# ZhengmaoHe/PARC

Hardware: AMD Instinct MI355X
Metric: env-steps/sec (whole node), 4096 envs/GPU humanoid tracker at 1/2/4/8 MI355X (higher is better)
Workload: dtype f32; 1 GPU; 4096 envs/GPU tracker on procgen box heightfields, 64 synthetic clips (BASELINE.json configs[2]); envs_per_gpu=4096, env_steps_per_bench_step=131072, rollout_steps=32, update_epochs=5, minibatch=16384, sim_substeps=4, parallelism=dp1, scaling_rule=per-rank work fixed (T = 32, minibatch = 4 x envs): weak scaling, grad_allreduce=per minibatch (reference cadence)

## Files before the change

include/parc_hip.h:

```cpp
#ifndef PARC_HIP_H
#define PARC_HIP_H

#include <stdint.h>

#ifdef __cplusplus
extern "C" {
#endif

#define PARC_MAX_BODIES 16
#define PARC_MAX_DOFS 64
#define PARC_MAX_TAR_STEPS 6
#define PARC_MAX_KEY_BODIES 8

#define PARC_OK 0
#define PARC_EINVAL (-1)
#define PARC_EUNSUPPORTED (-2)

#define PARC_JOINT_ROOT 0
#define PARC_JOINT_HINGE 1
#define PARC_JOINT_SPHERICAL 2
#define PARC_JOINT_FIXED 3

#define PARC_DONE_NULL 0
#define PARC_DONE_FAIL 1
// ... 140 lines not shown
                               parc_track_cfg_t cfg, parc_env_buffers_t buf, const int64_t *env_ids, int n_sel, int what,
                               const float *ray_xy, void *start_event, void *stop_event);

int parc_assemble_obs(void *stream, int n_envs, const float *obs, int obs_dim, const float *aux, const float *scalar,
                      const int32_t *col_map, float *out, int out_dim, const int64_t *env_ids, int n_sel);

int parc_reset_apply(void *stream, int n_envs, const int32_t *mask, const int64_t *new_motion_ids, const int64_t *new_terrain_ids,
                     const float *new_time_offsets, const float *motion_offsets, int terrains_per_motion, int64_t *motion_ids,
                     int64_t *motion_terrain_ids, float *motion_time_offsets, float *motion_xy_offset, int32_t *timestep_buf,
                     float *time_buf, int32_t *done, float *next_target_time, int64_t *ep_num);

int parc_reset_sample_apply(void *stream, int n_envs, const int32_t *done_flags, int32_t *mask, const float *uniforms, int n_motions,
                            const float *motion_weights, const float *fail_rates, float min_weight, const float *motion_lengths,
                            const float *motion_offsets, int terrains_per_motion, float noise_scale, float *cdf_workspace,
                            int64_t *motion_ids, int64_t *motion_terrain_ids, float *motion_time_offsets, float *motion_xy_offset,
                            int32_t *timestep_buf, float *time_buf, int32_t *done, float *next_target_time, int64_t *ep_num,
                            float *init_noise_xy);

int parc_step_tail(void *stream, parc_char_model_t model, parc_motion_lib_t mlib, parc_env_buffers_t buf, int what, int n_motions,
                   const int32_t *done_kind, float ema_w, float *fail_rates);
int parc_update_fail_rates(void *stream, int n_envs, int n_motions, const int64_t *motion_ids, const int32_t *done_kind,
                           float ema_w, float *fail_rates);

int parc_td_lambda_return(void *stream, int T, int N, const float *reward, const float *next_vals, const int32_t *done,
                          float discount, float td_lambda, float *ret);
int parc_adv_normalize(void *stream, int n, const float *ret, const float *vals, const float *rand_action_mask,
                       float clip, float *norm_adv, float *mean_std_out , double *workspace);

typedef struct {
    float clip_ratio, bound_w, entropy_w, reg_w, critic_w, large_critic_loss;
    int32_t critic_l1;
} parc_ppo_cfg_t;
int parc_ppo_loss(void *stream, int B, int A, const float *mean, const float *logstd, const float *norm_a, const float *old_logp,
                  const float *adv, const float *mask, const float *pred, const float *tar_val, parc_ppo_cfg_t cfg, float *g_mean,
                  float *g_logstd, float *g_pred, float *out, float *workspace);
int parc_ppo_workspace_floats(int B);
int parc_ppo_loss_packed(void *stream, int B, int A, const float *mean, const float *logstd, const float *rec, int rec_stride,
                         const float *pred, parc_ppo_cfg_t cfg, float *g_mean, float *g_logstd, float *g_pred, float *out,
                         float *workspace);

typedef struct {
    const void *src;
    void *dst;
    int32_t row_bytes;
    int32_t convert;
} parc_record_field_t;
int parc_record_step(void *stream, int n_envs, const int64_t *head, int n_fields, const parc_record_field_t *fields);

int parc_rng_step(void *stream, uint64_t seed, uint64_t *state, float *uniform_out, int64_t n_uniform, float *normal_out, int64_t n_normal,
                  int64_t *tick_cell, int tick_mod);

int64_t parc_sgd_workspace_floats(void);
int parc_sgd_momentum_step(void *stream, int64_t n, float *params, const float *grad, float *momentum_buf, float max_norm, float lr,
                           float momentum, float weight_decay, float *workspace, float *norm_out);

int parc_adamw_step(void *stream, int64_t n, float *params, const float *grad, float *exp_avg, float *exp_avg_sq, int64_t step,
                    float max_norm, float lr, float beta1, float beta2, float eps, float weight_decay, float *workspace, float *norm_out);

int parc_normalize_clamp(void *stream, int64_t rows, int dim, const float *x, const float *mean, const float *stdv, float clip, float *out);

int64_t parc_moments_workspace_floats(int64_t rows, int dim);
int parc_moments_accumulate(void *stream, int64_t rows, int dim, const float *x, float *acc, float *workspace);
int parc_obs_ingest(void *stream, int64_t rows, int dim, const float *x, const float *mean, const float *stdv, float clip, float *norm_out,
                    float *copy_dst, const int64_t *copy_row, float *acc, float *workspace);

int parc_action_head(void *stream, int n, int A, const float *mean, const float *logstd, const float *noise, const float *explore,
                     const float *a_mean, const float *a_std, float *action, float *logp);
int parc_action_head_record(void *stream, int n, int A, const float *mean, const float *logstd, const float *noise, const float *explore,
                            const float *a_mean, const float *a_std, float *action, float *logp, float *rec_action, float *rec_logp,
                            float *rec_mask, const float *forces_src, float *rec_forces, int n_forces, const int64_t *head);

int parc_points_hf_sdf(void *stream, int batch, int n_points, int dim_x, int dim_y, const float *points, const float *hf,
                       const float *min_box_center, const float *x_points, const float *y_points, float half_x, float half_y,
                       float base_z, int inverted, float radius, float *out, int32_t *out_cell);

int parc_points_hf_sdf_grad(void *stream, int batch, int n_points, int dim_x, int dim_y, const float *points, const float *hf,
                            const float *min_box_center, const float *x_points, const float *y_points, float half_x, float half_y,
                            float base_z, int inverted, const int32_t *cell, const float *g_out, float *g_points);

int64_t parc_relu_bwd_workspace_floats(int64_t rows, int dim);
int parc_relu_bwd_bias_grad(void *stream, int64_t rows, int dim, float *gy, const float *y, float *db, float *workspace);
int parc_weighted_colsum(void *stream, int64_t rows, int dim, const float *x, const float *w, float *out, float *workspace);

int parc_abi_version(void);

#ifdef __cplusplus
}
#endif
#endif
```

parc_amd/_hip.py:

```python
import ctypes
import os
import subprocess

import torch

_HERE = os.path.dirname(os.path.abspath(__file__))
LIB_DIR = os.path.join(_HERE, "lib")
LIB_PATH = os.path.join(LIB_DIR, "libparc_hip.so")
CSRC = os.path.join(_HERE, "csrc")
SOURCES = ["parc_kin.hip", "parc_sim.hip", "parc_ppo.hip", "parc_rollout.hip", "parc_optim.hip", "parc_colreduce.hip", "parc_terrain.hip", "parc_render.hip", "parc_score.hip", "parc_netstats.hip", "parc_moopt.hip",
           "parc_augment.hip", "parc_mdm_batch.hip", "parc_hfgather.hip", "parc_motion.hip", "parc_pose_opt.hip", "parc_returns.hip"]
DIAG_LIB_PATH = os.path.join(LIB_DIR, "libparc_hip_diag.so")
DIAG_SOURCES = SOURCES + ["parc_sim_ref.hip"]

MAX_BODIES = 16
MAX_DOFS = 64
MAX_TAR_STEPS = 6
MAX_KEY_BODIES = 8

POST_REF = 1
POST_OBS = 2
POST_REWARD_DONE = 4
POST_HF = 8
POST_MASKED = 16
# ... 120 lines not shown
        objs.append(o)
    for cmd, p in procs:
        if p.wait() != 0:
            raise subprocess.CalledProcessError(p.returncode, cmd)
    cmd = [hipcc, "--offload-arch=gfx950", "-shared", "-fPIC", "-o", lib_path] + objs
    if verbose:
        print(" ".join(cmd))
    subprocess.check_call(cmd)
    with open(digest_path, "w") as f:
        f.write(digest + "\n")
    return lib_path


def lib():
    global _lib
    if _lib is None:
        if not os.path.exists(LIB_PATH):
            raise RuntimeError("libparc_hip.so is not built ({}); run `python -c 'import __graft_entry__ as g; g.build()'` "
                               "-- there is no CPU fallback".format(LIB_PATH))
        if _stored_digest() != source_digest():
            raise RuntimeError("libparc_hip.so was built from other sources than the ones beside it (csrc/, include/): rebuild with "
                               "`python -c 'import __graft_entry__ as g; g.build()'` - calling a stale library would hand it argument "
                               "structs of another layout")
        _lib = ctypes.CDLL(LIB_PATH)
        _declare(_lib)
    return _lib


def _declare(L):
    L.parc_abi_version.restype = c_int
    L.parc_refresh_ray_obs_hfs.argtypes = [c_vp, c_int, c_vp, c_int, c_vp, c_vp, TerrainS, c_f, c_f, c_vp, c_i64]
    L.parc_refresh_obs_hfs.argtypes = [c_vp, c_int, c_vp, c_int, c_vp, c_vp, TerrainS, c_f, c_f, c_vp, c_i64]
    L.parc_dof_to_rot.argtypes = [c_vp, CharModelS, c_int, c_vp, c_vp]
    L.parc_rot_to_dof.argtypes = [c_vp, CharModelS, c_int, c_vp, c_vp]
    L.parc_forward_kinematics.argtypes = [c_vp, CharModelS, c_int, c_vp, c_vp, c_vp, c_vp, c_vp]
    L.parc_pose_chain_forward.argtypes = [c_vp, CharModelS, c_int, c_vp, c_vp, c_vp, c_vp, c_vp, c_vp, c_vp]
    L.parc_pose_chain_backward.argtypes = [c_vp, CharModelS, c_int, c_vp, c_vp, c_vp, c_vp, c_vp, c_vp, c_vp, c_vp, c_vp]
    L.parc_body_points_world.argtypes = [c_vp, c_int, c_int, c_int, c_vp, c_vp, c_vp, c_vp, c_vp]
    L.parc_body_points_world_grad.argtypes = [c_vp, c_int, c_int, c_int, c_vp, c_vp, c_vp, c_vp, c_vp, c_vp]
    L.parc_quat_diff_angle.argtypes = [c_vp, ctypes.c_int64, c_vp, c_vp, c_vp]
    L.parc_quat_diff_angle_grad.argtypes = [c_vp, ctypes.c_int64, c_vp, c_vp, c_vp, c_vp, c_vp]
    L.parc_temporal_terms.argtypes = [c_vp, c_int, c_int, c_vp, c_vp, c_vp, c_vp, c_vp, c_f, c_f, c_f, c_vp]
    L.parc_temporal_terms_grad.argtypes = [c_vp, c_int, c_int, c_vp, c_vp, c_vp, c_vp, c_vp, c_f, c_f, c_f, c_vp, c_vp, c_vp]
    L.parc_calc_motion_frame.argtypes = [c_vp, MotionLibS, c_int, c_vp, c_vp] + [c_vp] * 7
    L.parc_motion_lib_build.argtypes = [c_vp, CharModelS, MotionLibS, c_int, c_vp, c_vp, c_vp, c_vp, c_vp]
    L.parc_track_post_step.argtypes = [c_vp, CharModelS, MotionLibS, TerrainS, TrackCfgS, EnvBuffersS, c_vp, c_int, c_int, c_vp]
    L.parc_track_post_step_timed.argtypes = L.parc_track_post_step.argtypes + [c_vp, c_vp]
    L.parc_track_post_step_timed.restype = c_int
    L.parc_assemble_obs.argtypes = [c_vp, c_int, c_vp, c_int, c_vp, c_vp, c_vp, c_vp, c_int, c_vp, c_int]
    L.parc_assemble_obs.restype = c_int
    L.parc_update_fail_rates.argtypes = [c_vp, c_int, c_int, c_vp, c_vp, c_f, c_vp]
    L.parc_step_tail.argtypes = [c_vp, CharModelS, MotionLibS, EnvBuffersS, c_int, c_int, c_vp, c_f, c_vp]
    L.parc_step_tail.restype = c_int
    L.parc_td_lambda_return.argtypes = [c_vp, c_int, c_int, c_vp, c_vp, c_vp, c_f, c_f, c_vp]
    L.parc_adv_normalize.argtypes = [c_vp, c_int, c_vp, c_vp, c_vp, c_f, c_vp, c_vp, c_vp]
    L.parc_ppo_loss.argtypes = [c_vp, c_int, c_int] + [c_vp] * 8 + [PPOCfgS] + [c_vp] * 5
    L.parc_ppo_loss.restype = c_int
    L.parc_ppo_loss_packed.argtypes = [c_vp, c_int, c_int, c_vp, c_vp, c_vp, c_int, c_vp, PPOCfgS] + [c_vp] * 5
    L.parc_ppo_loss_packed.restype = c_int
    L.parc_ppo_workspace_floats.argtypes = [c_int]
    L.parc_ppo_workspace_floats.restype = c_int
    L.parc_normalize_clamp.argtypes = [c_vp, c_i64, c_int, c_vp, c_vp, c_vp, c_f, c_vp]
    L.parc_normalize_clamp.restype = c_int
    L.parc_action_head.argtypes = [c_vp, c_int, c_int] + [c_vp] * 8
    L.parc_action_head.restype = c_int
    L.parc_action_head_record.argtypes = [c_vp, c_int, c_int] + [c_vp] * 8 + [c_vp] * 5 + [c_int, c_vp]
    L.parc_action_head_record.restype = c_int
    L.parc_points_hf_sdf.argtypes = [c_vp, c_int, c_int, c_int, c_int] + [c_vp] * 5 + [c_f, c_f, c_f, c_int, c_f, c_vp, c_vp]
    L.parc_points_hf_sdf.restype = c_int
    L.parc_points_hf_sdf_grad.argtypes = [c_vp, c_int, c_int, c_int, c_int] + [c_vp] * 5 + [c_f, c_f, c_f, c_int, c_vp, c_vp, c_vp]
    L.parc_points_hf_sdf_grad.restype = c_int
    L.parc_scale_by_clipped_norm.argtypes = [c_vp, c_i64, c_vp, c_vp, c_f]
    L.parc_scale_by_clipped_norm.restype = c_int
    L.parc_moments_workspace_floats.argtypes = [c_i64, c_int]
    L.parc_moments_workspace_floats.restype = c_i64
    L.parc_moments_accumulate.argtypes = [c_vp, c_i64, c_int, c_vp, c_vp, c_vp]
    L.parc_moments_accumulate.restype = c_int
    L.parc_relu_bwd_workspace_floats.argtypes = [c_i64, c_int]
    L.parc_relu_bwd_workspace_floats.restype = c_i64
    L.parc_relu_bwd_bias_grad.argtypes = [c_vp, c_i64, c_int, c_vp, c_vp, c_vp, c_vp]
    L.parc_relu_bwd_bias_grad.restype = c_int
    L.parc_weighted_colsum.argtypes = [c_vp, c_i64, c_int, c_vp, c_vp, c_vp, c_vp]
    L.parc_weighted_colsum.restype = c_int
    L.parc_sgd_workspace_floats.argtypes = []
    L.parc_sgd_workspace_floats.restype = c_i64
    L.parc_sgd_momentum_step.argtypes = [c_vp, c_i64, c_vp, c_vp, c_vp, c_f, c_f, c_f, c_f, c_vp, c_vp]
    L.parc_sgd_momentum_step.restype = c_int
    L.parc_adamw_step.argtypes = [c_vp, c_i64, c_vp, c_vp, c_vp, c_vp, c_i64, c_f, c_f, c_f, c_f, c_f, c_f, c_vp, c_vp]
    L.parc_adamw_step.restype = c_int
    L.parc_return_tracker_update.argtypes = [c_vp, c_int, c_int, c_vp, c_i64] + [c_vp] * 8
    L.parc_return_tracker_workspace_floats.argtypes = [c_int]
    L.parc_return_tracker_workspace_floats.restype = c_i64
    L.parc_return_tracker_update.restype = c_int
    L.parc_record_step.argtypes = [c_vp, c_int, c_vp, c_int, c_vp]
    L.parc_record_step.restype = c_int
    L.parc_obs_ingest.argtypes = [c_vp, c_i64, c_int, c_vp, c_vp, c_vp, c_f, c_vp, c_vp, c_vp, c_vp, c_vp]
    L.parc_obs_ingest.restype = c_int
    L.parc_rng_step.argtypes = [c_vp, ctypes.c_uint64, c_vp, c_vp, c_i64, c_vp, c_i64, c_vp, c_int]
    L.parc_rng_step.restype = c_int
    L.parc_reset_apply.argtypes = [c_vp, c_int, c_vp, c_vp, c_vp, c_vp, c_vp, c_int] + [c_vp] * 9
    L.parc_reset_apply.restype = c_int
    L.parc_reset_sample_apply.argtypes = [c_vp, c_int, c_vp, c_vp, c_vp, c_int, c_vp, c_vp, c_f, c_vp, c_vp, c_int, c_f] + [c_vp] * 11
    L.parc_reset_sample_apply.restype = c_int
    for name in ("parc_refresh_ray_obs_hfs", "parc_refresh_obs_hfs", "parc_dof_to_rot", "parc_rot_to_dof",
                 "parc_forward_kinematics", "parc_calc_motion_frame", "parc_motion_lib_build", "parc_track_post_step", "parc_reset_apply",
                 "parc_update_fail_rates", "parc_td_lambda_return", "parc_adv_normalize"):
        getattr(L, name).restype = c_int
    if hasattr(L, "parc_sim_abi"):
        from . import _hip_sim
        _hip_sim.declare(L)
    if hasattr(L, "parc_render_abi"):
        from . import _hip_render
        _hip_render.declare(L)
    if hasattr(L, "parc_score_abi"):
        from . import _hip_score
        _hip_score.declare(L)
    if hasattr(L, "parc_netstats_abi"):
        from . import _hip_netstats
        _hip_netstats.declare(L)
    if hasattr(L, "parc_moopt_abi"):
        from . import _hip_moopt
        _hip_moopt.declare(L)
    if hasattr(L, "parc_augment_abi"):
        from . import _hip_augment
        _hip_augment.declare(L)
    if hasattr(L, "parc_mdm_batch_abi"):
        from . import _hip_mdm_batch
        _hip_mdm_batch.declare(L)


EXPORTED = ["parc_abi_version", "parc_refresh_ray_obs_hfs", "parc_refresh_obs_hfs", "parc_dof_to_rot", "parc_rot_to_dof",
            "parc_forward_kinematics", "parc_calc_motion_frame", "parc_motion_lib_build", "parc_track_post_step",
            "parc_update_fail_rates", "parc_td_lambda_return", "parc_adv_normalize", "parc_reset_apply", "parc_ppo_loss", "parc_ppo_workspace_floats", "parc_record_step", "parc_return_tracker_update", "parc_normalize_clamp",
            "parc_action_head", "parc_points_hf_sdf", "parc_moments_workspace_floats", "parc_moments_accumulate", "parc_reset_sample_apply", "parc_return_tracker_workspace_floats", "parc_scale_by_clipped_norm", "parc_relu_bwd_workspace_floats",
            "parc_relu_bwd_bias_grad", "parc_ppo_loss_packed", "parc_weighted_colsum", "parc_sgd_workspace_floats", "parc_sgd_momentum_step", "parc_adamw_step",
            "parc_pose_chain_forward", "parc_pose_chain_backward", "parc_points_hf_sdf_grad", "parc_body_points_world", "parc_body_points_world_grad",
            "parc_quat_diff_angle", "parc_quat_diff_angle_grad", "parc_temporal_terms", "parc_temporal_terms_grad", "parc_step_tail",
            "parc_assemble_obs", "parc_track_post_step_timed", "parc_rng_step", "parc_obs_ingest", "parc_action_head_record",
            "parc_render", "parc_render_abi", "parc_motion_score", "parc_score_abi",
            "parc_netstats_workspace_floats", "parc_netstats_update", "parc_netstats_abs_colsum", "parc_netstats_dormant_count", "parc_netstats_abi",
            "parc_points_hf_sdf_ragged", "parc_points_hf_sdf_ragged_grad", "parc_temporal_terms_seg", "parc_temporal_terms_seg_grad",
            "parc_segment_sums", "parc_moopt_abi",
            "parc_augment_frames", "parc_augment_terrains", "parc_augment_localize", "parc_augment_abi",
            "parc_mdm_heightfields", "parc_mdm_windows", "parc_mdm_batch_abi"]


def check(rc, what):
    if rc != 0:
        raise RuntimeError("{} failed with code {} ({})".format(what, rc, "bad argument" if rc == -1 else "unsupported" if rc == -2 else "hipError"))


def stream():
    return c_vp(torch.cuda.current_stream().cuda_stream)


def ptr(t):
    if t is None:
        return c_vp(0)
    assert t.is_cuda, "HIP kernels need device tensors (no CPU fallback)"
    assert t.is_contiguous(), "tensor must be contiguous"
    return c_vp(t.data_ptr())


def terrain_struct(hf, min_point, dxdy):
    assert hf.dtype == torch.float32 and hf.is_contiguous() and hf.dim() == 2
    return TerrainS(ptr(hf), int(hf.shape[0]), int(hf.shape[1]), float(min_point[0]), float(min_point[1]),
                    float(dxdy[0]), float(dxdy[1]))


class HipEventPair:
    _rt = None

    def __init__(self):
        if HipEventPair._rt is None:
            HipEventPair._rt = ctypes.CDLL("libamdhip64.so")
        self.start, self.stop = c_vp(), c_vp()
        for ev in (self.start, self.stop):
            rc = HipEventPair._rt.hipEventCreate(ctypes.byref(ev))
            if rc != 0:
                raise RuntimeError("hipEventCreate -> %d" % rc)

    def elapsed_us(self):
        ms = ctypes.c_float()
        rc = HipEventPair._rt.hipEventElapsedTime(ctypes.byref(ms), self.start, self.stop)
        if rc != 0:
            raise RuntimeError("hipEventElapsedTime -> %d" % rc)
        return ms.value * 1e3

    def __del__(self):
        try:
            for ev in (self.start, self.stop):
                if ev:
                    HipEventPair._rt.hipEventDestroy(ev)
        except Exception:
            pass
```

parc_amd/csrc/parc_colreduce.hip:

```cpp
#include <hip/hip_runtime.h>
#include <stdint.h>

#include "../../include/parc_hip.h"
#include "parc_launch.h"
#include "parc_learner_math.h"

__global__ __launch_bounds__(256) void normalize_clamp_kernel(size_t n4, int dim4, const float4 *__restrict__ x, const float4 *__restrict__ mean,
                                                              const float4 *__restrict__ stdv, float clip, float4 *__restrict__ out) {
    for (size_t i = (size_t)blockIdx.x * blockDim.x + threadIdx.x; i < n4; i += (size_t)gridDim.x * blockDim.x) {
        const int c = (int)(i % (size_t)dim4);
        const float4 v = x[i], m = mean[c], s = stdv[c];
        float4 o;
        o.x = clamp_nan((v.x - m.x) / s.x, -clip, clip);
        o.y = clamp_nan((v.y - m.y) / s.y, -clip, clip);
        o.z = clamp_nan((v.z - m.z) / s.z, -clip, clip);
        o.w = clamp_nan((v.w - m.w) / s.w, -clip, clip);
        out[i] = o;
    }
}

extern "C" int parc_normalize_clamp(void *stream, int64_t rows, int dim, const float *x, const float *mean, const float *stdv, float clip,
                                    float *out) {
    if (rows < 0 || dim <= 0 || (dim & 3) || (((uintptr_t)x | (uintptr_t)mean | (uintptr_t)stdv | (uintptr_t)out) & 15)) return PARC_EINVAL;
    if (rows == 0) return PARC_OK;
// ... 138 lines not shown
    hipLaunchKernelGGL(moments_partial_kernel, g.grid, dim3(256), 0, (hipStream_t)stream, (int)rows, g.dim4, (const float4 *)x, (float4 *)workspace);
    launch_moments_final(stream, g, workspace, acc);
    PARC_CHECK_LAUNCH();
    return PARC_OK;
}

#define RB_ROWS 128
__global__ __launch_bounds__(256) void relu_bwd_bias_partial_kernel(int rows, int dim4, float4 *__restrict__ gy, const float4 *__restrict__ y,
                                                                    float4 *__restrict__ partial) {
    __shared__ float4 red[4][64];
    const col_chunk_t k = col_chunk(rows, RB_ROWS);
    const int rg = k.rg, c = k.c, r0 = k.r0, r1 = k.r1;
    float4 s = make_float4(0.f, 0.f, 0.f, 0.f);
    if (c < dim4) {
#pragma unroll 4
        for (int r = r0 + rg; r < r1; r += 4) {
            const size_t i = (size_t)r * dim4 + c;
            float4 g = gy[i];
            const float4 a = y[i];
            g.x = a.x <= 0.f ? 0.f : g.x; g.y = a.y <= 0.f ? 0.f : g.y; g.z = a.z <= 0.f ? 0.f : g.z; g.w = a.w <= 0.f ? 0.f : g.w;
            gy[i] = g;
            s.x += g.x; s.y += g.y; s.z += g.z; s.w += g.w;
        }
    }
    fold_store(red, s, k, dim4, partial);
}

__global__ __launch_bounds__(256) void colsum_final_kernel(int chunks, int dim, const float *__restrict__ partial, float *__restrict__ out) {
    const int c = blockIdx.x * blockDim.x + threadIdx.x;
    if (c >= dim) return;
    float t = 0.f;
#pragma unroll 16
    for (int k = 0; k < chunks; ++k) t += partial[(size_t)k * dim + c];
    out[c] = t;
}

__global__ __launch_bounds__(256) void weighted_colsum_partial_kernel(int rows, int dim4, const float4 *__restrict__ x, const float *__restrict__ w,
                                                                      float4 *__restrict__ partial) {
    __shared__ float4 red[4][64];
    const col_chunk_t k = col_chunk(rows, RB_ROWS);
    const int rg = k.rg, c = k.c, r0 = k.r0, r1 = k.r1;
    float4 s = make_float4(0.f, 0.f, 0.f, 0.f);
    if (c < dim4) {
#pragma unroll 4
        for (int r = r0 + rg; r < r1; r += 4) {
            const float4 v = x[(size_t)r * dim4 + c];
            const float wr = w[r];
            s.x = fmaf(wr, v.x, s.x); s.y = fmaf(wr, v.y, s.y); s.z = fmaf(wr, v.z, s.z); s.w = fmaf(wr, v.w, s.w);
        }
    }
    fold_store(red, s, k, dim4, partial);
}

static void launch_colsum_final(void *stream, const col_grid_t &g, int dim, const float *workspace, float *out) {
    hipLaunchKernelGGL(colsum_final_kernel, dim3((dim + 255) / 256), dim3(256), 0, (hipStream_t)stream, g.chunks, dim, workspace, out);
}

extern "C" int parc_weighted_colsum(void *stream, int64_t rows, int dim, const float *x, const float *w, float *out, float *workspace) {
    const col_grid_t g = col_chunk_grid(rows, dim, RB_ROWS, (uintptr_t)x | (uintptr_t)workspace, !x || !w || !out || !workspace);
    if (g.rc != PARC_OK) return g.rc;
    if (rows > 0)
        hipLaunchKernelGGL(weighted_colsum_partial_kernel, g.grid, dim3(256), 0, (hipStream_t)stream, (int)rows, g.dim4, (const float4 *)x, w,
                           (float4 *)workspace);
    launch_colsum_final(stream, g, dim, workspace, out);
    PARC_CHECK_LAUNCH();
    return PARC_OK;
}

extern "C" int64_t parc_relu_bwd_workspace_floats(int64_t rows, int dim) {
    if (rows < 0 || dim <= 0) return -1;
    return ((rows + RB_ROWS - 1) / RB_ROWS) * (int64_t)dim;
}

extern "C" int parc_relu_bwd_bias_grad(void *stream, int64_t rows, int dim, float *gy, const float *y, float *db, float *workspace) {
    const col_grid_t g = col_chunk_grid(rows, dim, RB_ROWS, (uintptr_t)gy | (uintptr_t)y | (uintptr_t)workspace, !gy || !y || !db || !workspace);
    if (g.rc != PARC_OK) return g.rc;
    if (rows > 0)
        hipLaunchKernelGGL(relu_bwd_bias_partial_kernel, g.grid, dim3(256), 0, (hipStream_t)stream, (int)rows, g.dim4, (float4 *)gy, (const float4 *)y,
                           (float4 *)workspace);
    launch_colsum_final(stream, g, dim, workspace, db);
    PARC_CHECK_LAUNCH();
    return PARC_OK;
}
```

parc_amd/learning/dm_ppo_agent.py:

```python
import enum
import os
import time

import numpy as np
import torch

from ..envs import base_env
from ..gym_spaces import Box
from ..util import mp_util
from ..util.logger import Logger
from . import dm_ppo_model, experience_buffer, mp_optimizer, normalizer, rl_util, unit_stats
from .dm_ppo_return_tracker import DMPPOReturnTracker
from .tracking_error_tracker import TrackingErrorTracker


class AgentMode(enum.Enum):
    TRAIN = 0
    TEST = 1


_LOSS_KEYS = ["norm_obs", "action", "a_logp", "tar_val", "adv", "rand_action_mask"]


def enable_tuned_gemms():
    import torch.cuda.tunable as tunable
    path = os.path.join(os.path.dirname(os.path.dirname(os.path.abspath(__file__))), "tunableop_results.csv")
    if not os.path.exists(path) or tunable.is_enabled():
        return
    tunable.set_filename(path, False)
    tunable.tuning_enable(False)
    if hasattr(tunable, "write_file_on_exit"):
        tunable.write_file_on_exit(False)
    tunable.enable(True)


class DMPPOAgent(torch.nn.Module):
    NAME = "DM_PPO"

    def __init__(self, config, env, device):
        super().__init__()
        self._env = env
        self._device = device
        self._iter = 0
        self._sample_count = 0
        self._config = config
        self._is_terrain_runner = env.NAME in ("ig_terrain_runner", "ig_parkour")
        self._has_target_task = env.NAME in ("ig_terrain_runner", "ig_deepmimic_terrain", "ig_parkour")
        self._load_params(config)
        self._build_normalizers()
        self._model = dm_ppo_model.DMPPOModel(config["model"], env)
        self.to(self._device)
        params = [p for p in self.parameters() if p.requires_grad]
        self._optimizer = mp_optimizer.MPOptimizer(config["optimizer"], params)
        self._build_exp_buffer(config)
        self._train_return_tracker = DMPPOReturnTracker(self.get_num_envs(), self._device, self._has_target_task)
        self._test_return_tracker = DMPPOReturnTracker(self.get_num_envs(), self._device, self._has_target_task)
        self._mode = AgentMode.TRAIN
        self._curr_obs = None
        self._curr_info = None
        self._ppo_cfg = None
        if str(self._device).startswith("cuda") and config.get("tuned_gemms", True):
            enable_tuned_gemms()
        self._use_hip_graph = bool(config.get("hip_graph_rollout", True)) and str(self._device).startswith("cuda")
        self._graphs = dict()
        self._graph_pool = None
        self._graph_warm = 0
        self._exp_prob_t = torch.ones([1, 1], dtype=torch.float32, device=self._device)
        self._head_t = torch.zeros([1], dtype=torch.int64, device=self._device)
        self._head_dev, self._exp_prob_dev = 0, 1.0
        self._compute_times = []
        self._replan_time_rows, self._replan_time_src = None, None
        self._ones_mask = None
        self._unit_stats = None
        self._unit_report = None
        if getattr(self._env, "_report_tracking_error", False):
            self._test_tracking_error_tracker = TrackingErrorTracker(self.get_num_envs(), self._device)

    @staticmethod
    def rollout_shape(config, num_procs):
        P = int(num_procs) if config.get("mp_scale_rollout", True) else 1
        return int(np.ceil(config["steps_per_iter"] / P)), int(np.ceil(config["batch_size"] / P))

    def _load_params(self, config):
        self._discount = config["discount"]
        self._iters_per_output = config["iters_per_output"]
        self._iters_per_checkpoint = config["iters_per_checkpoint"]
        self._normalizer_samples = config.get("normalizer_samples", np.inf)
        self._test_episodes = config["test_episodes"]
        self._steps_per_iter, self._batch_size = self.rollout_shape(config, mp_util.get_num_procs())
        self._update_epochs = config["update_epochs"]
        self._td_lambda = config["td_lambda"]
        self._ppo_clip_ratio = config["ppo_clip_ratio"]
        self._norm_adv_clip = config["norm_adv_clip"]
        self._action_bound_weight = config["action_bound_weight"]
        self._action_entropy_weight = config["action_entropy_weight"]
        self._action_reg_weight = config["action_reg_weight"]
        self._critic_loss_weight = config["critic_loss_weight"]
        self._exp_anneal_samples = config.get("exp_anneal_samples", np.inf)
        self._exp_prob_beg = config.get("exp_prob_beg", 1.0)
        self._exp_prob_end = config.get("exp_prob_end", 1.0)
        self._clip_grad_norm = config.get("clip_grad_norm", False)
        self._max_grad_norm = config.get("max_grad_norm", 0.5)
        self._critic_loss_type = config.get("critic_loss_type", "L2")
        self._log_unit_stats = bool(config.get("log_unit_stats", False))

    def _build_normalizers(self):
        obs_space = self._env.get_obs_space()
        shapes = self._env._compute_obs(ret_obs_shapes=True)
        idx, cur = [], 0
        for key in shapes:
            shape = shapes[key]["shape"]
            flat = shape[0] * shape[1] if len(shape) >= 2 else shape[0]
            if not shapes[key]["use_normalizer"]:
                idx.append(torch.arange(cur, cur + flat, dtype=torch.int64, device=self._device))
            cur += flat
        non_norm = torch.cat(idx) if idx else None
        self._obs_norm = normalizer.Normalizer(obs_space.shape, device=self._device, dtype=torch.float32, non_norm_indices=non_norm,
                                               clip=self._config["norm_obs_clip"])
        a_space = self._env.get_action_space()
        assert isinstance(a_space, Box)
        a_mean = torch.tensor(0.5 * (a_space.high + a_space.low), device=self._device, dtype=torch.float32)
        a_std = torch.tensor(0.5 * (a_space.high - a_space.low), device=self._device, dtype=torch.float32)
        self._a_norm = normalizer.Normalizer(a_mean.shape, device=self._device, init_mean=a_mean, init_std=a_std, dtype=torch.float32)

    def _build_exp_buffer(self, config):
        T, N, dev = self._steps_per_iter, self.get_num_envs(), self._device
        self._exp_buffer = experience_buffer.ExperienceBuffer(buffer_length=T, batch_size=N, device=dev)
        obs_dim = list(self._env.get_obs_space().shape)
        a_dim = list(self._env.get_action_space().shape)
        B = self._env._cfg.num_bodies if hasattr(self._env, "_cfg") else 15

        def add(name, shape, dtype=torch.float32):
            self._exp_buffer.add_buffer(name, torch.zeros([T, N] + shape, device=dev, dtype=dtype))
# ... 713 lines not shown
```

parc_amd/learning/dm_ppo_model.py:

```python
import enum

import numpy as np
import torch


class StdType(enum.Enum):
    FIXED = 0
    CONSTANT = 1
    VARIABLE = 2


class DistributionGaussianDiag:
    def __init__(self, mean, logstd):
        self._mean = mean
        self._logstd = logstd
        self._std_cache = None
        self._dim = mean.shape[-1]

    @property
    def _std(self):
        if self._std_cache is None:
            self._std_cache = torch.exp(self._logstd)
        return self._std_cache

# ... 41 lines not shown
        elif std_type == StdType.CONSTANT:
            self._logstd_net = torch.nn.Parameter(torch.full((out_size,), logstd, dtype=torch.float32), requires_grad=True)
        else:
            self._logstd_net = torch.nn.Linear(in_size, out_size)
            torch.nn.init.uniform_(self._logstd_net.weight, -init_output_scale, init_output_scale)
            torch.nn.init.constant_(self._logstd_net.bias, logstd)

    def forward(self, x):
        mean = self._mean_net(x)
        if self._std_type == StdType.VARIABLE:
            logstd = self._logstd_net(x)
        else:
            logstd = torch.broadcast_to(self._logstd_net, mean.shape)
        return DistributionGaussianDiag(mean=mean, logstd=logstd)


_NETS = {"fc_3layers_2048units": [2048, 1024, 512], "fc_3layers_1024units": [1024, 1024, 512], "fc_2layers_1024units": [1024, 512]}


class _LinearReLU(torch.autograd.Function):

    @staticmethod
    def forward(ctx, x, weight, bias):
        y = torch._addmm_activation(bias, x, weight.t(), use_gelu=False)
        ctx.save_for_backward(x, weight, y)
        return y

    @staticmethod
    def backward(ctx, gy):
        x, weight, y = ctx.saved_tensors
        g = torch.ops.aten.threshold_backward(gy, y, 0.0)
        gx = g.mm(weight) if ctx.needs_input_grad[0] else None
        gw = g.t().mm(x) if ctx.needs_input_grad[1] else None
        gb = g.sum(dim=0) if ctx.needs_input_grad[2] else None
        return gx, gw, gb


class FusedMLP(torch.nn.Sequential):

    def forward(self, x):
        mods = list(self)
        if not (x.is_cuda and x.dim() == 2 and x.dtype == torch.float32):
            return super().forward(x)
        i = 0
        while i < len(mods):
            m = mods[i]
            if isinstance(m, torch.nn.Linear) and i + 1 < len(mods) and isinstance(mods[i + 1], torch.nn.ReLU):
                if torch.is_grad_enabled() and (x.requires_grad or m.weight.requires_grad):
                    x = _LinearReLU.apply(x, m.weight, m.bias)
                else:
                    x = torch._addmm_activation(m.bias, x, m.weight.t(), use_gelu=False)
                i += 2
            else:
                x = m(x)
                i += 1
        return x


def build_net(name, in_size, activation):
    if name not in _NETS:
        raise NotImplementedError("net '{}' (the tracker default is fc_3layers_2048units)".format(name))
    layers = []
    for out_size in _NETS[name]:
        lin = torch.nn.Linear(in_size, out_size)
        torch.nn.init.zeros_(lin.bias)
        layers += [lin, activation()]
        in_size = out_size
    return FusedMLP(*layers), in_size


class DMPPOModel(torch.nn.Module):
    def __init__(self, config, env):
        super().__init__()
        self._activation = torch.nn.ReLU
        obs_dim = int(np.prod(env.get_obs_space().shape))
        a_dim = int(np.prod(env.get_action_space().shape))
        self._actor_layers, h = build_net(config["actor_net"], obs_dim, self._activation)
        self._action_dist = DistributionGaussianDiagBuilder(h, a_dim, std_type=StdType[config["actor_std_type"]],
                                                            init_std=config["action_std"],
                                                            init_output_scale=config["actor_init_output_scale"])
        self._critic_layers, hc = build_net(config["critic_net"], obs_dim, self._activation)
        self._critic_out = torch.nn.Linear(hc, 1)
        torch.nn.init.zeros_(self._critic_out.bias)

    def eval_actor(self, obs):
        return self._action_dist(self._actor_layers(obs))

    @torch.no_grad()
    def eval_actor_tapped(self, obs):
        acts = self._trunk_forward(self._actor_layers, obs)
        mnet = self._action_dist._mean_net
        mean = torch.addmm(mnet.bias, acts[-1], mnet.weight.t())
        return DistributionGaussianDiag(mean=mean, logstd=torch.broadcast_to(self._action_dist._logstd_net, mean.shape)), acts[1:]

    def supports_explicit_backward(self):
        def plain(seq):
            mods = list(seq)
            return len(mods) % 2 == 0 and all(isinstance(m, torch.nn.Linear) for m in mods[0::2]) and all(isinstance(m, torch.nn.ReLU) for m in mods[1::2]) \
                and all(m.out_features % 4 == 0 for m in mods[0::2])
        return plain(self._actor_layers) and plain(self._critic_layers) and self._action_dist._std_type != StdType.VARIABLE

    @staticmethod
    def _trunk_forward(seq, x):
        acts = [x]
        for lin in list(seq)[0::2]:
            x = torch._addmm_activation(lin.bias, x, lin.weight.t(), use_gelu=False)
            acts.append(x)
        return acts

    @torch.no_grad()
    def train_forward(self, norm_obs):
        a = self._trunk_forward(self._actor_layers, norm_obs)
        c = self._trunk_forward(self._critic_layers, norm_obs)
        mnet = self._action_dist._mean_net
        mean = torch.addmm(mnet.bias, a[-1], mnet.weight.t())
        pred = torch.addmm(self._critic_out.bias, c[-1], self._critic_out.weight.t()).squeeze(-1)
        return mean, self._action_dist._logstd_net, pred, (a, c)

    def _relu_bwd(self, d, y, db):
        from .. import _hip
        L = _hip.lib()
        need = int(L.parc_relu_bwd_workspace_floats(d.shape[0], d.shape[1]))
        ws = getattr(self, "_relu_ws", None)
        if ws is None or ws.numel() < need or ws.device != d.device:
            ws = self._relu_ws = torch.empty(max(need, 1), dtype=torch.float32, device=d.device)
        _hip.check(L.parc_relu_bwd_bias_grad(_hip.stream(), d.shape[0], d.shape[1], _hip.ptr(d), _hip.ptr(y), _hip.ptr(db), _hip.ptr(ws)),
                   "parc_relu_bwd_bias_grad")

    def _weighted_colsum(self, x, w, out):
        from .. import _hip
        L = _hip.lib()
        need = int(L.parc_relu_bwd_workspace_floats(x.shape[0], x.shape[1]))
        ws = getattr(self, "_relu_ws", None)
        if ws is None or ws.numel() < need or ws.device != x.device:
            ws = self._relu_ws = torch.empty(max(need, 1), dtype=torch.float32, device=x.device)
        _hip.check(L.parc_weighted_colsum(_hip.stream(), x.shape[0], x.shape[1], _hip.ptr(x), _hip.ptr(w.contiguous()), _hip.ptr(out), _hip.ptr(ws)),
                   "parc_weighted_colsum")

    def _trunk_backward(self, seq, acts, d, grad_of, done):
        lins = list(seq)[0::2]
        for k in range(len(lins) - 1, -1, -1):
            lin = lins[k]
            self._relu_bwd(d, acts[k + 1], grad_of(lin.bias))
            torch.mm(d.t(), acts[k], out=grad_of(lin.weight))
            done(lin.weight)
            done(lin.bias)
            if k > 0:
                d = torch.mm(d, lin.weight)

    @torch.no_grad()
    def train_backward(self, saved, g_mean, g_logstd, g_pred, grad_of, done=lambda p: None):
        a, c = saved
        mnet = self._action_dist._mean_net
        torch.mm(g_mean.t(), a[-1], out=grad_of(mnet.weight))
        torch.sum(g_mean, dim=0, out=grad_of(mnet.bias))
        done(mnet.weight)
        done(mnet.bias)
        if self._action_dist._std_type == StdType.CONSTANT:
            grad_of(self._action_dist._logstd_net).copy_(g_logstd)
            done(self._action_dist._logstd_net)
        self._trunk_backward(self._actor_layers, a, torch.mm(g_mean, mnet.weight), grad_of, done)
        gp = g_pred.unsqueeze(-1)
        if self._critic_out.weight.shape[0] == 1:
            self._weighted_colsum(c[-1], g_pred, grad_of(self._critic_out.weight).view(-1))
        else:
            torch.mm(gp.t(), c[-1], out=grad_of(self._critic_out.weight))
        torch.sum(gp, dim=0, out=grad_of(self._critic_out.bias))
        done(self._critic_out.weight)
        done(self._critic_out.bias)
        self._trunk_backward(self._critic_layers, c, torch.mm(gp, self._critic_out.weight), grad_of, done)

    def eval_critic(self, obs):
        return self._critic_out(self._critic_layers(obs))
```

Before: 452,600 env-steps/s.

## Fuse value and policy head backward with top-layer ReLU bias grad

Adds HIP kernels that compute the output-head weight and bias gradients, the input gradient through the last ReLU, and the top hidden layer's bias gradient in one pass over the activations. The goal is to replace several separate launches (GEMV/mm, sum, mm, relu_bwd) for each head. The value-head fusion is enabled by default and the policy-head fusion is off by default. Workspaces are now kept per network, so actor and critic no longer share one buffer.

```diff
diff --git a/include/parc_hip.h b/include/parc_hip.h
--- a/include/parc_hip.h
+++ b/include/parc_hip.h
@@ -246,6 +246,12 @@
 int parc_relu_bwd_bias_grad(void *stream, int64_t rows, int dim, float *gy, const float *y, float *db, float *workspace);
 int parc_weighted_colsum(void *stream, int64_t rows, int dim, const float *x, const float *w, float *out, float *workspace);
 
+int64_t parc_head_bwd_workspace_floats(int64_t rows, int dim, int A);
+int parc_value_head_bwd(void *stream, int64_t rows, int dim, const float *y, const float *g_pred, const float *w_out, float *d, float *dW_out,
+                        float *db_out, float *db, float *workspace);
+int parc_policy_head_bwd(void *stream, int64_t rows, int dim, int A, const float *y, const float *g_mean, const float *W_mean, float *d,
+                         float *dW_mean, float *db_mean, float *db, float *workspace);
+
 int parc_abi_version(void);
 
 #ifdef __cplusplus
diff --git a/parc_amd/_hip.py b/parc_amd/_hip.py
--- a/parc_amd/_hip.py
+++ b/parc_amd/_hip.py
@@ -226,6 +226,12 @@
     L.parc_relu_bwd_bias_grad.restype = c_int
     L.parc_weighted_colsum.argtypes = [c_vp, c_i64, c_int, c_vp, c_vp, c_vp, c_vp]
     L.parc_weighted_colsum.restype = c_int
+    L.parc_head_bwd_workspace_floats.argtypes = [c_i64, c_int, c_int]
+    L.parc_head_bwd_workspace_floats.restype = c_i64
+    L.parc_value_head_bwd.argtypes = [c_vp, c_i64, c_int] + [c_vp] * 8
+    L.parc_value_head_bwd.restype = c_int
+    L.parc_policy_head_bwd.argtypes = [c_vp, c_i64, c_int, c_int] + [c_vp] * 8
+    L.parc_policy_head_bwd.restype = c_int
     L.parc_sgd_workspace_floats.argtypes = []
     L.parc_sgd_workspace_floats.restype = c_i64
     L.parc_sgd_momentum_step.argtypes = [c_vp, c_i64, c_vp, c_vp, c_vp, c_f, c_f, c_f, c_f, c_vp, c_vp]
@@ -286,7 +292,8 @@
             "parc_points_hf_sdf_ragged", "parc_points_hf_sdf_ragged_grad", "parc_temporal_terms_seg", "parc_temporal_terms_seg_grad",
             "parc_segment_sums", "parc_moopt_abi",
             "parc_augment_frames", "parc_augment_terrains", "parc_augment_localize", "parc_augment_abi",
-            "parc_mdm_heightfields", "parc_mdm_windows", "parc_mdm_batch_abi"]
+            "parc_mdm_heightfields", "parc_mdm_windows", "parc_mdm_batch_abi",
+            "parc_head_bwd_workspace_floats", "parc_value_head_bwd", "parc_policy_head_bwd"]
 
 
 def check(rc, what):
diff --git a/parc_amd/csrc/parc_colreduce.hip b/parc_amd/csrc/parc_colreduce.hip
--- a/parc_amd/csrc/parc_colreduce.hip
+++ b/parc_amd/csrc/parc_colreduce.hip
@@ -244,3 +244,219 @@
     PARC_CHECK_LAUNCH();
     return PARC_OK;
 }
+
+#define HEAD_MAX_A 32
+
+__global__ __launch_bounds__(256) void value_head_bwd_partial_kernel(int rows, int dim, const float4 *__restrict__ y, const float *__restrict__ g_pred,
+                                                                     const float *__restrict__ w_out, float4 *__restrict__ d,
+                                                                     float4 *__restrict__ partial_b, float4 *__restrict__ partial_w,
+                                                                     float *__restrict__ partial_g) {
+    __shared__ float4 red[2][4][64];
+    const int dim4 = dim / 4;
+    const col_chunk_t k = col_chunk(rows, RB_ROWS);
+    const int rg = k.rg, c = k.c, r0 = k.r0, r1 = k.r1;
+    float4 sb = make_float4(0.f, 0.f, 0.f, 0.f), sw = sb;
+    if (c < dim4) {
+        const float4 w = make_float4(w_out[4 * c], w_out[4 * c + 1], w_out[4 * c + 2], w_out[4 * c + 3]);
+#pragma unroll 4
+        for (int r = r0 + rg; r < r1; r += 4) {
+            const size_t i = (size_t)r * dim4 + c;
+            const float4 a = y[i];
+            const float g = g_pred[r];
+            float4 o;
+            o.x = a.x <= 0.f ? 0.f : __fmul_rn(g, w.x); o.y = a.y <= 0.f ? 0.f : __fmul_rn(g, w.y);
+            o.z = a.z <= 0.f ? 0.f : __fmul_rn(g, w.z); o.w = a.w <= 0.f ? 0.f : __fmul_rn(g, w.w);
+            d[i] = o;
+            sb.x += o.x; sb.y += o.y; sb.z += o.z; sb.w += o.w;
+            sw.x = fmaf(g, a.x, sw.x); sw.y = fmaf(g, a.y, sw.y); sw.z = fmaf(g, a.z, sw.z); sw.w = fmaf(g, a.w, sw.w);
+        }
+    }
+    fold_store(red[0], sb, k, dim4, partial_b);
+    fold_store(red[1], sw, k, dim4, partial_w);
+    if (blockIdx.x == 0 && rg == 1) {
+        double s = 0.0;
+        for (int r = r0 + k.lane; r < r1; r += 64) s += (double)g_pred[r];
+#pragma unroll
+        for (int o = 32; o >= 1; o >>= 1) s += __shfl_xor(s, o, 64);
+        if (k.lane == 0) partial_g[blockIdx.y] = (float)s;
+    }
+}
+
+template <int A4>
+__global__ __launch_bounds__(256) void policy_head_bwd_partial_kernel(int rows, int dim, int A, const float4 *__restrict__ y,
+                                                                      const float *__restrict__ g_mean, const float *__restrict__ W_mean,
+                                                                      float4 *__restrict__ d, float4 *__restrict__ partial_b,
+                                                                      float4 *__restrict__ partial_w, float *__restrict__ partial_g) {
+    constexpr int AP = 4 * A4, STAGED = AP * 64 + RB_ROWS * A4, FOLD = 4 * 4 * 64;
+    __shared__ float4 smem[STAGED > FOLD ? STAGED : FOLD];
+    float4 (*w_s)[64] = reinterpret_cast<float4 (*)[64]>(smem);
+    float4 (*g_s)[A4] = reinterpret_cast<float4 (*)[A4]>(smem + AP * 64);
+    const int dim4 = dim / 4;
+    const col_chunk_t k = col_chunk(rows, RB_ROWS);
+    const int lane = k.lane, rg = k.rg, c = k.c, r0 = k.r0, r1 = k.r1;
+    {
+        float *wf = reinterpret_cast<float *>(w_s), *gf = reinterpret_cast<float *>(g_s);
+        const int col0 = blockIdx.x * 256;
+        const int col = col0 + (int)threadIdx.x;
+        float wv[AP], gv[AP / 2];
+#pragma unroll
+        for (int a = 0; a < AP; ++a) {
+            const bool in = a < A && col < dim;
+            const float v = W_mean[in ? (size_t)a * dim + col : (size_t)0];
+            wv[a] = in ? v : 0.f;
+        }
+#pragma unroll
+        for (int j = 0; j < AP / 2; ++j) {
+            const int i = j * 256 + (int)threadIdx.x, r = r0 + i / AP, a = i % AP;
+            const bool in = r < r1 && a < A;
+            const float v = g_mean[in ? (size_t)r * A + a : (size_t)0];
+            gv[j] = in ? v : 0.f;
+        }
+#pragma unroll
+        for (int a = 0; a < AP; ++a) wf[a * 256 + threadIdx.x] = wv[a];
+#pragma unroll
+        for (int j = 0; j < AP / 2; ++j) gf[j * 256 + threadIdx.x] = gv[j];
+    }
+    static_assert(RB_ROWS == 128, "the staging loop above takes RB_ROWS * AP / 256 = AP / 2 elements per thread");
+    __syncthreads();
+    if (blockIdx.x == 0 && threadIdx.x < A) {
+        const float *gf = reinterpret_cast<const float *>(g_s);
+        double s = 0.0;
+        for (int i = 0; i < RB_ROWS; ++i) s += (double)gf[i * AP + threadIdx.x];
+        partial_g[(size_t)blockIdx.y * A + threadIdx.x] = (float)s;
+    }
+    float4 acc[AP];
+#pragma unroll
+    for (int a = 0; a < AP; ++a) acc[a] = make_float4(0.f, 0.f, 0.f, 0.f);
+    float4 sb = make_float4(0.f, 0.f, 0.f, 0.f);
+    if (c < dim4) {
+        float4 a_next = r0 + rg < r1 ? y[(size_t)(r0 + rg) * dim4 + c] : sb;
+        for (int r = r0 + rg; r < r1; r += 4) {
+            const size_t i = (size_t)r * dim4 + c;
+            const float4 a = a_next;
+            if (r + 4 < r1) a_next = y[i + (size_t)4 * dim4];
+            const float4 *gr = g_s[r - r0];
+            float4 o = make_float4(0.f, 0.f, 0.f, 0.f);
+#pragma unroll
+            for (int q = 0; q < A4; ++q) {
+                const float4 g4 = gr[q];
+                const float gq[4] = {g4.x, g4.y, g4.z, g4.w};
+#pragma unroll
+                for (int j = 0; j < 4; ++j) {
+                    const float g = gq[j];
+                    const float4 w = w_s[4 * q + j][lane];
+                    float4 &s = acc[4 * q + j];
+                    o.x = fmaf(g, w.x, o.x); o.y = fmaf(g, w.y, o.y); o.z = fmaf(g, w.z, o.z); o.w = fmaf(g, w.w, o.w);
+                    s.x = fmaf(g, a.x, s.x); s.y = fmaf(g, a.y, s.y); s.z = fmaf(g, a.z, s.z); s.w = fmaf(g, a.w, s.w);
+                }
+            }
+            o.x = a.x <= 0.f ? 0.f : o.x; o.y = a.y <= 0.f ? 0.f : o.y; o.z = a.z <= 0.f ? 0.f : o.z; o.w = a.w <= 0.f ? 0.f : o.w;
+            d[i] = o;
+            sb.x += o.x; sb.y += o.y; sb.z += o.z; sb.w += o.w;
+        }
+    }
+    float4 (*red)[4][64] = reinterpret_cast<float4 (*)[4][64]>(smem);
+#pragma unroll
+    for (int q = 0; q <= A4; ++q) {
+        __syncthreads();
+#pragma unroll
+        for (int j = 0; j < 4; ++j)
+            if (4 * q + j <= AP) red[rg][j][lane] = 4 * q + j < AP ? acc[4 * q + j < AP ? 4 * q + j : 0] : sb;
+        __syncthreads();
+        const int arr = 4 * q + rg;
+        if (c < dim4 && (arr < A || arr == AP)) {
+            const float4 s0 = red[0][rg][lane], s1 = red[1][rg][lane], s2 = red[2][rg][lane], s3 = red[3][rg][lane];
+            float4 o;
+            o.x = (s0.x + s1.x) + (s2.x + s3.x); o.y = (s0.y + s1.y) + (s2.y + s3.y);
+            o.z = (s0.z + s1.z) + (s2.z + s3.z); o.w = (s0.w + s1.w) + (s2.w + s3.w);
+            if (arr == AP) partial_b[(size_t)blockIdx.y * dim4 + c] = o;
+            else partial_w[((size_t)blockIdx.y * A + arr) * dim4 + c] = o;
+        }
+    }
+}
+
+__global__ __launch_bounds__(256) void head_bwd_final_kernel(int chunks, int dim, int A, const float *__restrict__ partial, float *__restrict__ db,
+                                                              float *__restrict__ dW, float *__restrict__ dbh) {
+    const int i = blockIdx.x * blockDim.x + threadIdx.x, n_w = (A + 1) * dim;
+    if (i < n_w) {
+        const bool is_w = i >= dim;
+        const int j = is_w ? i - dim : i;
+        const float *p = partial + (is_w ? (size_t)chunks * dim : (size_t)0);
+        const size_t stride = is_w ? (size_t)A * dim : (size_t)dim;
+        float t = 0.f;
+#pragma unroll 16
+        for (int k = 0; k < chunks; ++k) t += p[(size_t)k * stride + j];
+        (is_w ? dW : db)[j] = t;
+    } else if (i < n_w + A) {
+        const int a = i - n_w;
+        const float *p = partial + (size_t)chunks * n_w;
+        double t = 0.0;
+#pragma unroll 16
+        for (int k = 0; k < chunks; ++k) t += (double)p[(size_t)k * A + a];
+        dbh[a] = (float)t;
+    }
+}
+
+extern "C" int64_t parc_head_bwd_workspace_floats(int64_t rows, int dim, int A) {
+    if (rows < 0 || dim <= 0 || A < 1) return -1;
+    return (((rows + RB_ROWS - 1) / RB_ROWS) * ((int64_t)(A + 1) * dim + A) + 3) & ~(int64_t)3;
+}
+
+struct head_ws_t {
+    float *b, *w, *g;
+};
+
+static head_ws_t head_workspace(float *workspace, const col_grid_t &g, int dim, int A) {
+    float *w = workspace + (size_t)g.chunks * dim;
+    return {workspace, w, w + (size_t)g.chunks * A * dim};
+}
+
+static void launch_head_bwd_final(void *stream, const col_grid_t &g, int dim, int A, const float *workspace, float *db, float *dW, float *dbh) {
+    hipLaunchKernelGGL(head_bwd_final_kernel, dim3(((A + 1) * dim + A + 255) / 256), dim3(256), 0, (hipStream_t)stream, g.chunks, dim, A, workspace,
+                       db, dW, dbh);
+}
+
+extern "C" int parc_value_head_bwd(void *stream, int64_t rows, int dim, const float *y, const float *g_pred, const float *w_out, float *d,
+                                   float *dW_out, float *db_out, float *db, float *workspace) {
+    const col_grid_t g = col_chunk_grid(rows, dim, RB_ROWS, (uintptr_t)y | (uintptr_t)d | (uintptr_t)workspace,
+                                        !y || !g_pred || !w_out || !d || !dW_out || !db_out || !db || !workspace);
+    if (g.rc != PARC_OK) return g.rc;
+    const head_ws_t ws = head_workspace(workspace, g, dim, 1);
+    if (rows > 0)
+        hipLaunchKernelGGL(value_head_bwd_partial_kernel, g.grid, dim3(256), 0, (hipStream_t)stream, (int)rows, dim, (const float4 *)y, g_pred, w_out,
+                           (float4 *)d, (float4 *)ws.b, (float4 *)ws.w, ws.g);
+    launch_head_bwd_final(stream, g, dim, 1, workspace, db, dW_out, db_out);
+    PARC_CHECK_LAUNCH();
+    return PARC_OK;
+}
+
+template <int A4>
+static void launch_policy_head_bwd_partial(void *stream, const col_grid_t &g, int rows, int dim, int A, const float *y, const float *g_mean,
+                                           const float *W_mean, float *d, const head_ws_t &ws) {
+    hipLaunchKernelGGL(policy_head_bwd_partial_kernel<A4>, g.grid, dim3(256), 0, (hipStream_t)stream, rows, dim, A, (const float4 *)y, g_mean, W_mean,
+                       (float4 *)d, (float4 *)ws.b, (float4 *)ws.w, ws.g);
+}
+
+extern "C" int parc_policy_head_bwd(void *stream, int64_t rows, int dim, int A, const float *y, const float *g_mean, const float *W_mean, float *d,
+                                    float *dW_mean, float *db_mean, float *db, float *workspace) {
+    const col_grid_t g = col_chunk_grid(rows, dim, RB_ROWS, (uintptr_t)y | (uintptr_t)d | (uintptr_t)workspace,
+                                        A < 1 || !y || !g_mean || !W_mean || !d || !dW_mean || !db_mean || !db || !workspace);
+    if (g.rc != PARC_OK) return g.rc;
+    if (A > HEAD_MAX_A) return PARC_EUNSUPPORTED;
+    const head_ws_t ws = head_workspace(workspace, g, dim, A);
+    if (rows > 0) {
+        switch ((A + 3) / 4) {
+        case 1: launch_policy_head_bwd_partial<1>(stream, g, (int)rows, dim, A, y, g_mean, W_mean, d, ws); break;
+        case 2: launch_policy_head_bwd_partial<2>(stream, g, (int)rows, dim, A, y, g_mean, W_mean, d, ws); break;
+        case 3: launch_policy_head_bwd_partial<3>(stream, g, (int)rows, dim, A, y, g_mean, W_mean, d, ws); break;
+        case 4: launch_policy_head_bwd_partial<4>(stream, g, (int)rows, dim, A, y, g_mean, W_mean, d, ws); break;
+        case 5: launch_policy_head_bwd_partial<5>(stream, g, (int)rows, dim, A, y, g_mean, W_mean, d, ws); break;
+        case 6: launch_policy_head_bwd_partial<6>(stream, g, (int)rows, dim, A, y, g_mean, W_mean, d, ws); break;
+        case 7: launch_policy_head_bwd_partial<7>(stream, g, (int)rows, dim, A, y, g_mean, W_mean, d, ws); break;
+        default: launch_policy_head_bwd_partial<8>(stream, g, (int)rows, dim, A, y, g_mean, W_mean, d, ws); break;
+        }
+    }
+    launch_head_bwd_final(stream, g, dim, A, workspace, db, dW_mean, db_mean);
+    PARC_CHECK_LAUNCH();
+    return PARC_OK;
+}
diff --git a/parc_amd/learning/dm_ppo_agent.py b/parc_amd/learning/dm_ppo_agent.py
--- a/parc_amd/learning/dm_ppo_agent.py
+++ b/parc_amd/learning/dm_ppo_agent.py
@@ -49,6 +49,8 @@
         self._load_params(config)
         self._build_normalizers()
         self._model = dm_ppo_model.DMPPOModel(config["model"], env)
+        self._model.fused_head_backward = bool(config.get("fused_head_backward", True))
+        self._model.fused_policy_head_backward = bool(config.get("fused_policy_head_backward", False))
         self.to(self._device)
         params = [p for p in self.parameters() if p.requires_grad]
         self._optimizer = mp_optimizer.MPOptimizer(config["optimizer"], params)
diff --git a/parc_amd/learning/dm_ppo_model.py b/parc_amd/learning/dm_ppo_model.py
--- a/parc_amd/learning/dm_ppo_model.py
+++ b/parc_amd/learning/dm_ppo_model.py
@@ -147,6 +147,9 @@
         self._critic_layers, hc = build_net(config["critic_net"], obs_dim, self._activation)
         self._critic_out = torch.nn.Linear(hc, 1)
         torch.nn.init.zeros_(self._critic_out.bias)
+        self.fused_head_backward = True
+        self.fused_policy_head_backward = False
+        self._ws = {}
 
     def eval_actor(self, obs):
         return self._action_dist(self._actor_layers(obs))
@@ -182,31 +185,65 @@
         pred = torch.addmm(self._critic_out.bias, c[-1], self._critic_out.weight.t()).squeeze(-1)
         return mean, self._action_dist._logstd_net, pred, (a, c)
 
-    def _relu_bwd(self, d, y, db):
+    def _workspace(self, net, need, device):
+        ws = self._ws.get(net)
+        if ws is None or ws.numel() < need or ws.device != device:
+            ws = self._ws[net] = torch.empty(max(need, 1), dtype=torch.float32, device=device)
+        return ws
+
+    def _relu_bwd(self, d, y, db, net):
         from .. import _hip
         L = _hip.lib()
-        need = int(L.parc_relu_bwd_workspace_floats(d.shape[0], d.shape[1]))
-        ws = getattr(self, "_relu_ws", None)
-        if ws is None or ws.numel() < need or ws.device != d.device:
-            ws = self._relu_ws = torch.empty(max(need, 1), dtype=torch.float32, device=d.device)
+        ws = self._workspace(net, int(L.parc_relu_bwd_workspace_floats(d.shape[0], d.shape[1])), d.device)
         _hip.check(L.parc_relu_bwd_bias_grad(_hip.stream(), d.shape[0], d.shape[1], _hip.ptr(d), _hip.ptr(y), _hip.ptr(db), _hip.ptr(ws)),
                    "parc_relu_bwd_bias_grad")
 
-    def _weighted_colsum(self, x, w, out):
+    def _weighted_colsum(self, x, w, out, net):
         from .. import _hip
         L = _hip.lib()
-        need = int(L.parc_relu_bwd_workspace_floats(x.shape[0], x.shape[1]))
-        ws = getattr(self, "_relu_ws", None)
-        if ws is None or ws.numel() < need or ws.device != x.device:
-            ws = self._relu_ws = torch.empty(max(need, 1), dtype=torch.float32, device=x.device)
+        ws = self._workspace(net, int(L.parc_relu_bwd_workspace_floats(x.shape[0], x.shape[1])), x.device)
         _hip.check(L.parc_weighted_colsum(_hip.stream(), x.shape[0], x.shape[1], _hip.ptr(x), _hip.ptr(w.contiguous()), _hip.ptr(out), _hip.ptr(ws)),
                    "parc_weighted_colsum")
 
-    def _trunk_backward(self, seq, acts, d, grad_of, done):
+    HEAD_BWD_MAX_A = 32
+
+    def _head_bwd(self, net, y, g, weight, d, dw, dbh, db):
+        from .. import _hip
+        L = _hip.lib()
+        rows, dim = y.shape
+        A = 1 if g.dim() == 1 else g.shape[1]
+        ws = self._workspace(net, int(L.parc_head_bwd_workspace_floats(rows, dim, A)), y.device)
+        p = _hip.ptr
+        if g.dim() == 1:
+            _hip.check(L.parc_value_head_bwd(_hip.stream(), rows, dim, p(y), p(g), p(weight.view(-1)), p(d), p(dw.view(-1)), p(dbh), p(db), p(ws)),
+                       "parc_value_head_bwd")
+        else:
+            _hip.check(L.parc_policy_head_bwd(_hip.stream(), rows, dim, A, p(y), p(g), p(weight), p(d), p(dw), p(dbh), p(db), p(ws)),
+                       "parc_policy_head_bwd")
+
+    def _net_backward(self, net, seq, acts, head, g, grad_of, done, head_done):
         lins = list(seq)[0::2]
-        for k in range(len(lins) - 1, -1, -1):
+        y, top = acts[-1], len(lins) - 1
+        A = 1 if g.dim() == 1 else g.shape[1]
+        fused = self.fused_head_backward if g.dim() == 1 else self.fused_policy_head_backward
+        if fused and head.weight.shape[0] == A and A <= self.HEAD_BWD_MAX_A and g.is_contiguous() and y.is_contiguous():
+            d = torch.empty_like(y)
+            self._head_bwd(net, y, g, head.weight, d, grad_of(head.weight), grad_of(head.bias), grad_of(lins[top].bias))
+        else:
+            g2 = g if g.dim() == 2 else g.unsqueeze(-1)
+            if g.dim() == 1 and head.weight.shape[0] == 1:
+                self._weighted_colsum(y, g, grad_of(head.weight).view(-1), net)
+            else:
+                torch.mm(g2.t(), y, out=grad_of(head.weight))
+            torch.sum(g2, dim=0, out=grad_of(head.bias))
+            d = torch.mm(g2, head.weight)
+            self._relu_bwd(d, y, grad_of(lins[top].bias), net)
+        for p in head_done:
+            done(p)
+        for k in range(top, -1, -1):
             lin = lins[k]
-            self._relu_bwd(d, acts[k + 1], grad_of(lin.bias))
+            if k < top:
+                self._relu_bwd(d, acts[k + 1], grad_of(lin.bias), net)
             torch.mm(d.t(), acts[k], out=grad_of(lin.weight))
             done(lin.weight)
             done(lin.bias)
@@ -217,23 +254,13 @@
     def train_backward(self, saved, g_mean, g_logstd, g_pred, grad_of, done=lambda p: None):
         a, c = saved
         mnet = self._action_dist._mean_net
-        torch.mm(g_mean.t(), a[-1], out=grad_of(mnet.weight))
-        torch.sum(g_mean, dim=0, out=grad_of(mnet.bias))
-        done(mnet.weight)
-        done(mnet.bias)
+        head_done = [mnet.weight, mnet.bias]
         if self._action_dist._std_type == StdType.CONSTANT:
             grad_of(self._action_dist._logstd_net).copy_(g_logstd)
-            done(self._action_dist._logstd_net)
-        self._trunk_backward(self._actor_layers, a, torch.mm(g_mean, mnet.weight), grad_of, done)
-        gp = g_pred.unsqueeze(-1)
-        if self._critic_out.weight.shape[0] == 1:
-            self._weighted_colsum(c[-1], g_pred, grad_of(self._critic_out.weight).view(-1))
-        else:
-            torch.mm(gp.t(), c[-1], out=grad_of(self._critic_out.weight))
-        torch.sum(gp, dim=0, out=grad_of(self._critic_out.bias))
-        done(self._critic_out.weight)
-        done(self._critic_out.bias)
-        self._trunk_backward(self._critic_layers, c, torch.mm(gp, self._critic_out.weight), grad_of, done)
+            head_done.append(self._action_dist._logstd_net)
+        self._net_backward("actor", self._actor_layers, a, mnet, g_mean, grad_of, done, head_done)
+        self._net_backward("critic", self._critic_layers, c, self._critic_out, g_pred, grad_of, done,
+                           [self._critic_out.weight, self._critic_out.bias])
 
     def eval_critic(self, obs):
         return self._critic_out(self._critic_layers(obs))
```

Measured after the change: 455,000 env-steps/s (median of 6 runs). No clear change (+0.5%).
